# menmitsu/opticalFlowClustering

Measured on AMD Instinct MI355X. Metric: Mpixels/s dense flow+kmeans @1080p, higher is better.
Workload: dtype f32 storage, f64 accumulation; 1 GPU; BASELINE.json configs[2]: 300-frame 1080p synthetic clip, Farneback flow (0.5,3,15,3,5,1.2,0) + Lloyd k=5 over (u,v), frames sharded over 1 GPU(s); width=1920, height=1080, frames=300, pairs=299, k=5, lloyd_iters=11, flow_batch_pairs=64

## Files before the change

include/ofc.h:

```cpp
#ifndef OFC_H
#define OFC_H
#include <stddef.h>
#include <stdint.h>

#ifdef __cplusplus
extern "C" {
#endif

#define OFC_VERSION 100

enum {
    OFC_OK = 0,
    OFC_EINVAL = -1,
    OFC_ENODEV = -2,
    OFC_EHIP = -3,
    OFC_ENOMEM = -4,
    OFC_ENOTREADY = -5,
    OFC_EUNSUPPORTED = -6,
    OFC_ECOMM = -7
};

enum { OFC_U8 = 0, OFC_F32 = 1, OFC_F64 = 2 };

int ofc_version(void);
// ... 15 lines not shown
    int poly_n;
    double poly_sigma;
    int flags;
} ofc_fb_params;
#define OFC_WINSIZE_MAX 255

void ofc_fb_default_params(ofc_fb_params *p);

typedef struct ofc_flow ofc_flow_t;

int ofc_flow_create(int device, int W, int H, const ofc_fb_params *p, int max_batch,
                    ofc_flow_t **out);
void ofc_flow_destroy(ofc_flow_t *f);

int ofc_flow_calc(ofc_flow_t *f, const uint8_t *prev_gray, const uint8_t *next_gray,
                  float *flow_out);

int ofc_flow_calc_frames_dev(ofc_flow_t *f, const uint8_t *frames_dev, int n_frames,
                             float *flow_dev);
int ofc_flow_calc_frames_dev_stats(ofc_flow_t *f, const uint8_t *frames_dev, int n_frames,
                                   float *flow_dev, double *uv_sum_dev);
int ofc_flow_sync(ofc_flow_t *f);
int ofc_flow_front_overlap(const ofc_flow_t *f, int *on);

int ofc_flow_push_gray(ofc_flow_t *f, const uint8_t *gray, float *flow_out);

int ofc_flow_push_bgr(ofc_flow_t *f, const uint8_t *bgr, uint8_t *vis_out, float *mean_mag,
                      float *flow_out);
int ofc_flow_last_vis_dev(ofc_flow_t *f, const uint8_t **vis_dev);

int ofc_level_image(int device, const uint8_t *gray, int W, int H, const ofc_fb_params *p, int k,
                    float *out, int *w_out, int *h_out);
int ofc_polyexp(int device, const float *img, int W, int H, int n, double sigma, float *R5);
int ofc_polyexp_u8(int device, const uint8_t *gray, int W, int H, int n, double sigma, float *R5);
int ofc_update_matrices(int device, const float *R0, const float *R1, const float *flow, int W,
                        int H, float *M);
int ofc_box_solve(int device, const float *M, int W, int H, int winsize, float *flow);
int ofc_flow_resize(int device, const float *flow, int sw, int sh, int dw, int dh, float mul,
                    float *out);

int ofc_flow_iterate(int device, const float *R0, const float *R1, const float *flow_in, int W, int H,
                     int winsize, int iters, int mode, int rows_per_block, float *flow_out);
int ofc_flow_launch_geometry(int W, int H, int n_pairs, int winsize, int out[3]);
int ofc_bench_flow_iters(int device, int W, int H, int n_pairs, int reps, int mode, float *ms);

int ofc_bench_polyexp(int device, int W, int H, int n_images, int iters, int rows_per_block,
                      float *ms_per_launch);

int ofc_bgr2gray(int device, const uint8_t *bgr, int W, int H, uint8_t *gray);
int ofc_flow_to_bgr(int device, const float *flow, int W, int H, uint8_t *bgr, float *mean_mag);
int ofc_flow_to_bgr_dev(int device, const float *flow_dev, int W, int H, int n_frames,
                        uint8_t *bgr_dev, float *mean_mag_dev);
int ofc_bgr2hsv(int device, const uint8_t *bgr, int64_t npix, uint8_t *hsv);
int ofc_preprocess_rgba(int device, const uint8_t *img3, int64_t npix, int thresh, uint8_t *rgba);
int ofc_grid_cell_means(int device, const uint8_t *bgr, int W, int H, int rows, int cols,
// ... 224 lines not shown
```

opticalflowclustering_amd/_lib.py:

```python
import ctypes as C
import os

import numpy as np

_HERE = os.path.dirname(os.path.abspath(__file__))
LIB_PATH = os.path.join(_HERE, "libofc.so")

OFC_OK, OFC_EINVAL, OFC_ENODEV, OFC_EHIP, OFC_ENOMEM, OFC_ENOTREADY, OFC_EUNSUPPORTED, OFC_ECOMM = \
    0, -1, -2, -3, -4, -5, -6, -7
U8, F32, F64 = 0, 1, 2
UNIQUE_ID_BYTES = 128
KPP_CHUNK = 1024
UV_HIST_SHARE = 2048
UV_HIST_MAX_GRID = 2048
BLOB_TILE_W, BLOB_TILE_H, BLOB_FIELDS = 64, 16, 12
BLOB_LINK_FIELDS, BLOB_NO_MOVE = 3, -0x7fff8000
CONSIST_OK, CONSIST_MISMATCH, CONSIST_LEAVES, CONSIST_INVALID, CONSIST_STATES = 0, 1, 2, 3, 4
CONSIST_SHARE, CONSIST_MAX_DIM = 2048, 16384
CONSIST_ALPHA_MAX, CONSIST_BETA_MAX = 65536, 1 << 62
PHOTO_SHARE, PHOTO_TAU_MAX, PHOTO_KAPPA_MAX, PHOTO_NSTAT = 2048, 65280, 1024, 5
REPAIR_ROUNDS_MAX, REPAIR_NCOUNT, REPAIR_UNFILLED = 254, 3, 255


class OfcError(RuntimeError):
# ... 14 lines not shown

_lib = None

_vp, _i, _i64, _f, _d, _sz = C.c_void_p, C.c_int, C.c_int64, C.c_float, C.c_double, C.c_size_t
_ip = C.POINTER(C.c_int)
_PROTOS = {
    "ofc_version": ([], _i),
    "ofc_last_error": ([], C.c_char_p),
    "ofc_device_count": ([_ip], _i),
    "ofc_malloc": ([_i, _sz, C.POINTER(_vp)], _i),
    "ofc_free": ([_i, _vp], _i),
    "ofc_memcpy_h2d": ([_i, _vp, _vp, _sz], _i),
    "ofc_memcpy_d2h": ([_i, _vp, _vp, _sz], _i),
    "ofc_memset": ([_i, _vp, _i, _sz], _i),
    "ofc_device_sync": ([_i], _i),
    "ofc_fb_default_params": ([C.POINTER(FbParams)], None),
    "ofc_flow_create": ([_i, _i, _i, C.POINTER(FbParams), _i, C.POINTER(_vp)], _i),
    "ofc_flow_destroy": ([_vp], None),
    "ofc_flow_calc": ([_vp, _vp, _vp, _vp], _i),
    "ofc_flow_calc_frames_dev": ([_vp, _vp, _i, _vp], _i),
    "ofc_flow_calc_frames_dev_stats": ([_vp, _vp, _i, _vp, _vp], _i),
    "ofc_flow_sync": ([_vp], _i),
    "ofc_flow_front_overlap": ([_vp, _ip], _i),
    "ofc_flow_push_gray": ([_vp, _vp, _vp], _i),
    "ofc_flow_push_bgr": ([_vp, _vp, _vp, C.POINTER(_f), _vp], _i),
    "ofc_flow_last_vis_dev": ([_vp, C.POINTER(_vp)], _i),
    "ofc_level_image": ([_i, _vp, _i, _i, C.POINTER(FbParams), _i, _vp, _ip, _ip], _i),
    "ofc_polyexp": ([_i, _vp, _i, _i, _i, _d, _vp], _i),
    "ofc_polyexp_u8": ([_i, _vp, _i, _i, _i, _d, _vp], _i),
    "ofc_update_matrices": ([_i, _vp, _vp, _vp, _i, _i, _vp], _i),
    "ofc_box_solve": ([_i, _vp, _i, _i, _i, _vp], _i),
    "ofc_flow_resize": ([_i, _vp, _i, _i, _i, _i, _f, _vp], _i),
    "ofc_flow_iterate": ([_i, _vp, _vp, _vp, _i, _i, _i, _i, _i, _i, _vp], _i),
    "ofc_flow_launch_geometry": ([_i, _i, _i, _i, _ip], _i),
    "ofc_bench_flow_iters": ([_i, _i, _i, _i, _i, _i, C.POINTER(_f)], _i),
    "ofc_bench_polyexp": ([_i, _i, _i, _i, _i, _i, C.POINTER(_f)], _i),
    "ofc_bgr2gray": ([_i, _vp, _i, _i, _vp], _i),
    "ofc_flow_to_bgr": ([_i, _vp, _i, _i, _vp, C.POINTER(_f)], _i),
    "ofc_flow_to_bgr_dev": ([_i, _vp, _i, _i, _i, _vp, _vp], _i),
    "ofc_bgr2hsv": ([_i, _vp, _i64, _vp], _i),
    "ofc_preprocess_rgba": ([_i, _vp, _i64, _i, _vp], _i),
    "ofc_grid_cell_means": ([_i, _vp, _i, _i, _i, _i, _vp, _vp], _i),
    "ofc_kmeans_fit": ([_i, _vp, _i, _i64, _i, _i, _vp, _i, _d, _vp, _vp, C.POINTER(_d), _ip], _i),
    "ofc_kmeans_predict": ([_i, _vp, _i, _i64, _i, _i, _vp, _vp], _i),
    "ofc_kmeans_fit_dev": ([_i, _vp, _i, _i64, _i, _i, _vp, _i, _d, _vp, _vp, C.POINTER(_d), _ip], _i),
    "ofc_kmeans_fit_dev_stats": ([_i, _vp, _i, _i64, _i, _i, _vp, _i, _d, _vp, _vp, _vp, C.POINTER(_d), _ip], _i),
    "ofc_kmeans_fit_dev_field": ([_i, _vp, _i, _i64, _i, _i, _vp, _i, _d, _vp, _vp, _vp, C.POINTER(_d), _ip, _i, _i, _i64], _i),
    "ofc_lloyd_field_origin": ([_i64, _i, _i], _i64),
    "ofc_lloyd_field_origins": ([_i64, _i64, _i, _vp], _i),
    "ofc_lloyd_field_shape": ([_ip, _ip, _ip, _ip], None),
    "ofc_lloyd_prune_stats": ([_i, _vp], _i),
    "ofc_bench_lloyd_sweep": ([_i, _vp, _i64, _i, _vp, _vp, _i, _i, C.POINTER(_f)], _i),
    "ofc_lloyd_colstats_dev": ([_i, _vp, _i, _i64, _i, _vp, _i, _vp], _i),
    "ofc_lloyd_step_dev": ([_i, _vp, _i, _i64, _i, _i, _vp, _vp, _vp, _i, _vp], _i),
    "ofc_lloyd_inertia_dev": ([_i, _vp, _i, _i64, _i, _i, _vp, _vp, _vp, C.POINTER(_d)], _i),
    "ofc_lloyd_farthest_dev": ([_i, _vp, _i, _i64, _i, _i, _vp, _vp, _vp, _vp, _i, C.POINTER(_d), C.POINTER(_i64), _vp, _ip], _i),
    "ofc_kmeans_fit_w": ([_i, _vp, _i, _vp, _i, _i64, _i, _i, _vp, _i, _d, _vp, _vp, C.POINTER(_d), _ip], _i),
# ... 157 lines not shown
```

opticalflowclustering_amd/csrc/flow_kernels.hip:

```cpp
#include "flow_device.h"

namespace ofc {

__device__ __forceinline__ void lin_tap_x(int dx, double scale, int sw, int &s0, float &a)
{
#pragma clang fp contract(off)
    float fx = (float)((dx + 0.5) * scale - 0.5);
    int sx = (int)floorf(fx);
    fx -= (float)sx;
    if (sx < 0) { fx = 0.f; sx = 0; }
    if (sx >= sw - 1) { fx = 0.f; sx = sw - 1; }
    s0 = sx;
    a = fx;
}

__device__ __forceinline__ void lin_tap_y(int dy, double scale, int sh, int &s0, int &s1, float &b)
{
#pragma clang fp contract(off)
    float fy = (float)((dy + 0.5) * scale - 0.5);
    int sy = (int)floorf(fy);
    fy -= (float)sy;
    s0 = min(max(sy, 0), sh - 1);
    s1 = min(max(sy + 1, 0), sh - 1);
    b = fy;
// ... 261 lines not shown
int launch_level_image(const uint8_t *src, float *dst, int nimg, int W0, int H0,
                       const LevelGeom &g, hipStream_t s)
{
    LevelArgs a;
    int path = 1;
    size_t lds = 0;
    OFC_TRY(level_image_plan(W0, H0, g, ((uintptr_t)src % 4) == 0, a, path, lds));
    switch (path) {
    case 0:
        hipLaunchKernelGGL(k_level0, dim3(cdiv(W0, 256), cdiv(H0, 32), nimg), dim3(256), 0, s, src, dst, W0, H0,
                           a.kern[0], a.kern[1], a.kern[2]);
        break;
#define OFC_DEC(S_, R_, TX_, TY_)                                                                          \
    case S_:                                                                                               \
        hipLaunchKernelGGL((k_level_dec<S_, R_, TX_, TY_>), dim3(cdiv(g.w, TX_), cdiv(g.h, TY_), nimg),    \
                           dim3(256), 0, s, src, dst, W0, H0, g.w, g.h, a);                                \
        break;
    OFC_DEC(2, 1, 64, 16)
    OFC_DEC(4, 4, 32, 8)
    OFC_DEC(8, 9, 32, 8)
#undef OFC_DEC
    default:
        hipLaunchKernelGGL(k_level_image, dim3(cdiv(g.w, a.txo), cdiv(g.h, a.tyo), nimg), dim3(256), lds, s, src, dst, a);
    }
    OFC_HIP(hipGetLastError());
    return OFC_OK;
}

__device__ __forceinline__ float4 lds_read4(const float *p)
{
    typedef float v4f __attribute__((ext_vector_type(4)));
    typedef const volatile v4f __attribute__((address_space(3))) * lds_v4f_ptr;
    const v4f v = *(lds_v4f_ptr)(p);
    return make_float4(v.x, v.y, v.z, v.w);
}

constexpr int PE_TX = 240;
constexpr int PE_CH = 8;
constexpr int PE_PLANE = 78;

template <int N>
struct PolyArgs {
    int W, H, rows_per_block;
    float g[N + 1], xg[N + 1], xxg[N + 1];
    double ig11, ig03, ig33, ig55;
};
// ... 1104 lines not shown
```

opticalflowclustering_amd/csrc/ofc_api.cpp:

```cpp
#include "color_common.h"
#include "host_util.h"
#include "lloyd_common.h"

#include <cfloat>
#include <algorithm>
#include <cmath>
#include <cstdlib>
#include <memory>

namespace ofc {

static thread_local std::string g_err;

void set_error(const char *fmt, ...)
{
    char buf[1024];
    va_list ap;
    va_start(ap, fmt);
    vsnprintf(buf, sizeof(buf), fmt, ap);
    va_end(ap);
    g_err = buf;
}

int ensure_device(int device)
// ... 175 lines not shown
}

void ofc_fb_default_params(ofc_fb_params *p)
{
    if (!p) return;
    p->pyr_scale = 0.5; p->levels = 3; p->winsize = 15; p->iterations = 3;
    p->poly_n = 5; p->poly_sigma = 1.2; p->flags = 0;
}

}

struct ofc_flow {
    int device = 0, W = 0, H = 0, max_batch = 0, levels = 0;
    ofc_fb_params prm{};
    PolyConsts pc{};
    std::vector<LevelGeom> geom;
    hipStream_t stream = nullptr;
    DevBuf I, R, M, flowA, flowB, flowC;
    bool front_overlap = false;
    hipStream_t side = nullptr;
    hipEvent_t fork = nullptr;
    std::vector<hipEvent_t> ready;
    std::vector<size_t> offI, offR;
    bool fused = true;
    bool fuse_level0 = true;
    bool fuse2 = false;
    int fuse2_min_w = 0;
    bool w3 = false;
    int w3_min_w = 0;
    DevBuf frames2, flow1;
    DevBuf prev_gray;
    bool have_prev = false;
    DevBuf bgr_in, vis, vis_partial, vis_stats, mean_mag;
    bool have_vis = false;
    DevBuf uv_scratch;
    struct Captured {
        const uint8_t *frames = nullptr;
        int n_frames = 0;
        float *flow = nullptr;
        double *uv_sum = nullptr;
        int hits = 0;
        hipGraph_t graph = nullptr;
        hipGraphExec_t exec = nullptr;
    };
    std::vector<Captured> graphs;
    bool use_graph = false;
};

namespace ofc {

static int flow_run(ofc_flow *f, const uint8_t *frames_dev, int n_frames, float *flow_dev, double *uv_sum_dev = nullptr)
{
    const int npair = n_frames - 1;
    const int W = f->W, H = f->H;
    hipStream_t s = f->stream;
    const int iters = f->prm.iterations;
    float *prevFlow = nullptr;
    int pw = 0, ph = 0;
    auto front_end = [&](int k, hipStream_t st) -> int {
        float *I = f->I.as<float>() + f->offI[k], *R = f->R.as<float>() + f->offR[k];
        const LevelGeom &g = f->geom[k];
        if (k == 0 && f->fuse_level0 && polyexp_u8_ok(W, H, g)) return launch_polyexp_u8(frames_dev, R, n_frames, W, H, f->pc, st);
        OFC_TRY(launch_level_image(frames_dev, I, n_frames, W, H, g, st));
        return launch_polyexp(I, R, n_frames, g.w, g.h, f->pc, 0, st);
    };
    if (f->front_overlap) {
        OFC_HIP(hipEventRecord(f->fork, s));
        OFC_HIP(hipStreamWaitEvent(f->side, f->fork, 0));
        for (int k = f->levels; k >= 1; k--) {
            OFC_TRY(front_end(k, f->side));
            OFC_HIP(hipEventRecord(f->ready[k], f->side));
        }
        OFC_TRY(front_end(0, s));
    }
    for (int k = f->levels; k >= 0; k--) {
        const LevelGeom &g = f->geom[k];
        const size_t P = (size_t)g.w * g.h;
        float *dst = (k == 0) ? flow_dev : (((f->levels - k) & 1) ? f->flowB.as<float>() : f->flowA.as<float>());
        float *tmp = f->flowC.as<float>();
        const float *R = f->R.as<float>() + f->offR[k];
        if (!f->front_overlap) {
            OFC_TRY(front_end(k, s));
        } else if (k >= 1) {
            OFC_HIP(hipStreamWaitEvent(s, f->ready[k], 0));
        }
        const size_t strideR = 5 * P;
        const float mul = (float)(1. / f->prm.pyr_scale);
        if (f->fused) {
            const bool two = f->fuse2 && f->prm.winsize == 15 && g.w >= f->fuse2_min_w;
            int plan[64], L = 0;
            for (int i = 0; i < iters;) {
                const int n = (two && i > 0 && iters - i >= 2) ? 2 : 1;
                plan[L++] = n;
// ... 142 lines not shown
    OFC_HIP(hipStreamCreateWithFlags(&f->stream, hipStreamNonBlocking));
    const size_t P0 = (size_t)W * H, nb = (size_t)max_batch;
    size_t nI = P0 * (nb + 1), nR = 5 * P0 * (nb + 1);
    f->offI.assign(f->levels + 1, 0);
    f->offR.assign(f->levels + 1, 0);
    {
        const bool u8_level0 = f->fuse_level0 && polyexp_u8_ok(W, H, f->geom[0]);
        std::vector<size_t> oI(f->levels + 1, 0), oR(f->levels + 1, 0);
        size_t sI = 0, sR = 0;
        for (int k = 0; k <= f->levels; k++) {
            const size_t Pk = (size_t)f->geom[k].w * f->geom[k].h;
            oR[k] = sR;
            sR += (5 * Pk * (nb + 1) + 63) & ~(size_t)63;
            oI[k] = sI;
            if (k > 0 || !u8_level0) sI += (Pk * (nb + 1) + 63) & ~(size_t)63;
        }
        const char *eo = getenv("OFC_FLOW_FRONT_OVERLAP");
        f->front_overlap = !(eo && eo[0] == '0') && f->levels >= 1 && !f->use_graph && 2 * (sI + sR) <= 3 * (nI + nR);
        if (f->front_overlap) {
            f->offI = oI; f->offR = oR;
            nI = sI; nR = sR;
        }
    }
    if (f->front_overlap) {
        OFC_HIP(hipStreamCreateWithFlags(&f->side, hipStreamNonBlocking));
        OFC_HIP(hipEventCreateWithFlags(&f->fork, hipEventDisableTiming));
        f->ready.assign(f->levels + 1, nullptr);
        for (int k = 1; k <= f->levels; k++) OFC_HIP(hipEventCreateWithFlags(&f->ready[k], hipEventDisableTiming));
    }
    OFC_TRY(f->I.alloc(sizeof(float) * nI));
    OFC_TRY(f->R.alloc(sizeof(float) * nR));
    if (f->fused) {
        OFC_TRY(f->flowC.alloc(sizeof(float) * 2 * P0 * nb));
    } else {
        OFC_TRY(f->M.alloc(sizeof(float) * 5 * P0 * nb));
    }
    const size_t P1 = f->levels >= 1 ? (size_t)f->geom[1].w * f->geom[1].h : 1;
    OFC_TRY(f->flowA.alloc(sizeof(float) * 2 * P1 * nb));
    OFC_TRY(f->flowB.alloc(sizeof(float) * 2 * P1 * nb));
    OFC_TRY(f->frames2.alloc(2 * P0));
    OFC_TRY(f->flow1.alloc(sizeof(float) * 2 * P0));
    OFC_TRY(f->prev_gray.alloc(P0));
    *out = f.release();
    return OFC_OK;
}

// ... 30 lines not shown
    OFC_REQUIRE(n_frames >= 2 && n_frames - 1 <= f->max_batch, "n_frames-1 = %d pairs not in [1, max_batch=%d]",
                n_frames - 1, f->max_batch);
    OFC_TRY(ensure_device(f->device));
    return flow_run_cached(f, frames_dev, n_frames, flow_dev, uv_sum_dev);
}

hipStream_t ofc_flow_stream_internal(ofc_flow_t *f) { return f->stream; }

int ofc_flow_sync(ofc_flow_t *f)
{
    OFC_REQUIRE(f, "null pointer");
    OFC_TRY(ensure_device(f->device));
    OFC_HIP(hipStreamSynchronize(f->stream));
    return OFC_OK;
}

int ofc_flow_front_overlap(const ofc_flow_t *f, int *on)
{
    OFC_REQUIRE(f && on, "null pointer");
    *on = f->front_overlap ? 1 : 0;
    return OFC_OK;
}

int ofc_flow_calc(ofc_flow_t *f, const uint8_t *prev_gray, const uint8_t *next_gray, float *flow_out)
{
    OFC_REQUIRE(f && prev_gray && next_gray && flow_out, "null pointer");
    OFC_TRY(ensure_device(f->device));
    const size_t P0 = (size_t)f->W * f->H;
    uint8_t *fr = f->frames2.as<uint8_t>();
    OFC_HIP(hipMemcpyAsync(fr, prev_gray, P0, hipMemcpyHostToDevice, f->stream));
    OFC_HIP(hipMemcpyAsync(fr + P0, next_gray, P0, hipMemcpyHostToDevice, f->stream));
    OFC_TRY(flow_run(f, fr, 2, f->flow1.as<float>()));
    OFC_HIP(hipMemcpyAsync(flow_out, f->flow1.p, sizeof(float) * 2 * P0, hipMemcpyDeviceToHost, f->stream));
    OFC_HIP(hipStreamSynchronize(f->stream));
    return OFC_OK;
}

int ofc_flow_push_gray(ofc_flow_t *f, const uint8_t *gray, float *flow_out)
{
    OFC_REQUIRE(f && gray, "null pointer");
    OFC_TRY(ensure_device(f->device));
    const size_t P0 = (size_t)f->W * f->H;
    uint8_t *fr = f->frames2.as<uint8_t>();
    if (!f->have_prev) {
        OFC_HIP(hipMemcpyAsync(f->prev_gray.p, gray, P0, hipMemcpyHostToDevice, f->stream));
        OFC_HIP(hipStreamSynchronize(f->stream));
// ... 64 lines not shown
{
    for (int c = 0; c < 5; c++)
        for (size_t i = 0; i < P; i++) planar[c * P + i] = inter[i * 5 + c];
}

int ofc_level_image(int device, const uint8_t *gray, int W, int H, const ofc_fb_params *p, int k,
                    float *out, int *w_out, int *h_out)
{
    OFC_REQUIRE(gray && out, "null pointer");
    ofc_fb_params prm;
    if (p) prm = *p; else ofc_fb_default_params(&prm);
    OFC_TRY(check_params(prm, W, H));
    OFC_REQUIRE(k >= 0 && k <= pyramid_levels(W, H, prm), "level %d out of range", k);
    OFC_TRY(ensure_device(device));
    LevelGeom g = level_geometry(W, H, prm, k);
    DevBuf src, dst;
    OFC_TRY(src.alloc((size_t)W * H));
    OFC_TRY(dst.alloc(sizeof(float) * g.w * g.h));
    OFC_HIP(hipMemcpy(src.p, gray, (size_t)W * H, hipMemcpyHostToDevice));
    OFC_TRY(launch_level_image(src.as<uint8_t>(), dst.as<float>(), 1, W, H, g, nullptr));
    OFC_HIP(hipMemcpy(out, dst.p, sizeof(float) * g.w * g.h, hipMemcpyDeviceToHost));
    if (w_out) *w_out = g.w;
    if (h_out) *h_out = g.h;
    return OFC_OK;
}

int ofc_polyexp(int device, const float *img, int W, int H, int n, double sigma, float *R5)
{
    OFC_REQUIRE(img && R5, "null pointer");
    OFC_REQUIRE(W >= 1 && H >= 1, "bad size");
    OFC_TRY(polyexp_n_check(n));
    OFC_TRY(ensure_device(device));
    const size_t P = (size_t)W * H;
    PolyConsts pc;
    polyexp_setup(n, sigma, pc);
    DevBuf I, R;
    OFC_TRY(I.alloc(sizeof(float) * P));
    OFC_TRY(R.alloc(sizeof(float) * 5 * P));
    OFC_HIP(hipMemcpy(I.p, img, sizeof(float) * P, hipMemcpyHostToDevice));
    OFC_TRY(launch_polyexp(I.as<float>(), R.as<float>(), 1, W, H, pc, 0, nullptr));
    OFC_HIP(hipMemcpy(R5, R.p, sizeof(float) * 5 * P, hipMemcpyDeviceToHost));
    return OFC_OK;
}

int ofc_polyexp_u8(int device, const uint8_t *gray, int W, int H, int n, double sigma, float *R5)
{
// ... 171 lines not shown
    PolyConsts pc;
    polyexp_setup(5, 1.2, pc);
    DevBuf I, R;
    OFC_TRY(I.alloc(sizeof(float) * P * n_images));
    OFC_TRY(R.alloc(sizeof(float) * 5 * P * n_images));
    {
        std::vector<float> h(P);
        uint32_t st = 12345u;
        for (int im = 0; im < n_images; im++) {
            for (size_t i = 0; i < P; i++) {
                st = st * 1664525u + 1013904223u;
                h[i] = (float)(st >> 24);
            }
            OFC_HIP(hipMemcpy(I.as<float>() + (size_t)im * P, h.data(), sizeof(float) * P, hipMemcpyHostToDevice));
        }
    }
    ScopedStream own;
    OFC_TRY(own.create());
    hipStream_t s = own.s;
    auto launch = [&]() -> int { return launch_polyexp(I.as<float>(), R.as<float>(), n_images, W, H, pc, rows_per_block, s, true); };
    return time_launches(s, iters, launch, ms_per_launch);
}

}
```

opticalflowclustering_amd/csrc/ofc_common.h:

```cpp
#pragma once
#include <hip/hip_runtime.h>
#include <cstdarg>
#include <cstdint>
#include <cstdio>
#include <cstring>
#include <string>
#include <vector>

#include "../../include/ofc.h"

namespace ofc {

void set_error(const char *fmt, ...);
int ensure_device(int device);

#define OFC_HIP(expr)                                                                         \
    do {                                                                                      \
        hipError_t _e = (expr);                                                               \
        if (_e != hipSuccess) {                                                               \
            ofc::set_error("%s failed: %s (%s:%d)", #expr, hipGetErrorString(_e), __FILE__,   \
                           __LINE__);                                                         \
            return _e == hipErrorOutOfMemory ? OFC_ENOMEM : OFC_EHIP;                         \
        }                                                                                     \
    } while (0)
// ... 37 lines not shown
};

static inline int cdiv(int a, int b) { return (a + b - 1) / b; }
static inline int64_t cdiv64(int64_t a, int64_t b) { return (a + b - 1) / b; }

struct LevelGeom {
    int w, h, ksize;
    double sigma;
};
int pyramid_levels(int W, int H, const ofc_fb_params &p);
LevelGeom level_geometry(int W, int H, const ofc_fb_params &p, int k);
void gaussian_kernel(int n, double sigma, float *k);
struct PolyConsts {
    int n;
    float g[8], xg[8], xxg[8];
    double ig11, ig03, ig33, ig55;
};
void polyexp_setup(int n, double sigma, PolyConsts &c);
int polyexp_n_check(int n);
constexpr int WINSIZE_WIDE_MIN = 19;

int launch_level_image(const uint8_t *src, float *dst, int nimg, int W0, int H0,
                       const LevelGeom &g, hipStream_t s);
bool polyexp_u8_ok(int W, int H, const LevelGeom &g);
int launch_polyexp_u8(const uint8_t *frames, float *R, int nimg, int W, int H, const PolyConsts &c, hipStream_t s);
int launch_polyexp(const float *I, float *R, int nimg, int W, int H, const PolyConsts &c,
                   int rows_per_block, hipStream_t s, bool bench_tag = false);
int launch_update_matrices(const float *R0, const float *R1, size_t pair_stride_R,
                           const float *flow, float *M, int npair, int W, int H, hipStream_t s);
int launch_box_solve(const float *M, float *flow, int npair, int W, int H, int winsize,
                     int rows_per_block, hipStream_t s);
int launch_flow_resize(const float *src, float *dst, int npair, int sw, int sh, int dw, int dh,
                       float mul, hipStream_t s);
int launch_flow_iter(const float *R, size_t frame_stride_R, const float *flow_in, float *flow_out,
                     int npair, int W, int H, int winsize, hipStream_t s, const float *coarse = nullptr,
                     int sw = 0, int sh = 0, float mul = 1.f, double *uv_sum = nullptr, double *uv_scratch = nullptr,
                     size_t uv_scratch_doubles = 0, int rows_per_block = 0);
int flow_iter_rows(int W, int H, int npair, int winsize);
int flow_iter_max_grid(int W, int H, int npair, int winsize);
int launch_flow_iter2(const float *R, size_t frame_stride_R, const float *flow_in, float *flow_out, int npair, int W,
                      int H, int winsize, hipStream_t s, int rows_per_block = 0);
int launch_flow_iter_w3(const float *R, size_t frame_stride_R, const float *flow_in, float *flow_out, int npair, int W,
                        int H, int winsize, hipStream_t s, int rows_per_block = 0);
int launch_flow_iter_pipe(const float *R, size_t frame_stride_R, const float *flow_in, float *flow_out, int npair, int W,
                          int H, int rows_per_block, hipStream_t s, double *uv_sum, double *uv_scratch,
                          size_t uv_scratch_doubles);
// ... 9 lines not shown
```

opticalflowclustering_amd/flow.py:

```python
import ctypes as C
import threading
from collections import OrderedDict

import numpy as np

from . import _lib
from ._lib import FbParams, check, load, ptr


class FlowEngine:

    def __init__(self, W, H, params=None, max_batch=1, device=0):
        self.W, self.H, self.device, self.max_batch = int(W), int(H), device, int(max_batch)
        self.params = params or FbParams()
        h = C.c_void_p()
        check(load().ofc_flow_create(device, self.W, self.H, C.byref(self.params), self.max_batch, C.byref(h)))
        self._h = h

    def calc(self, prev_gray, next_gray, out=None):
        prev_gray = np.ascontiguousarray(prev_gray, np.uint8)
        next_gray = np.ascontiguousarray(next_gray, np.uint8)
        if prev_gray.shape != (self.H, self.W) or next_gray.shape != (self.H, self.W):
            raise ValueError(f"expected two {self.H}x{self.W} uint8 images")
        if out is None:
# ... 9 lines not shown
            raise ValueError(f"expected a {self.H}x{self.W} uint8 image")
        flow = np.empty((self.H, self.W, 2), np.float32)
        rc = load().ofc_flow_push_gray(self._h, ptr(gray), ptr(flow))
        if rc == _lib.OFC_ENOTREADY:
            return None
        check(rc)
        return flow

    def calc_frames_dev(self, frames_ptr, n_frames, flow_ptr, sync=True, uv_sum_ptr=None):
        if uv_sum_ptr:
            check(load().ofc_flow_calc_frames_dev_stats(self._h, C.c_void_p(frames_ptr), n_frames, C.c_void_p(flow_ptr),
                                                        C.c_void_p(uv_sum_ptr)))
        else:
            check(load().ofc_flow_calc_frames_dev(self._h, C.c_void_p(frames_ptr), n_frames, C.c_void_p(flow_ptr)))
        if sync:
            self.sync()

    def sync(self):
        check(load().ofc_flow_sync(self._h))

    def front_overlap(self):
        on = C.c_int(-1)
        check(load().ofc_flow_front_overlap(self._h, C.byref(on)))
        return bool(on.value)

    def close(self):
        if getattr(self, "_h", None):
            load().ofc_flow_destroy(self._h)
            self._h = None

    def __del__(self):
        try:
            self.close()
        except Exception:
            pass


def _is_flow_buffer(a, H, W):
    return (isinstance(a, np.ndarray) and a.dtype == np.float32 and a.shape == (H, W, 2)
            and a.flags.c_contiguous and a.flags.writeable)


OPTFLOW_USE_INITIAL_FLOW = 4
OPTFLOW_FARNEBACK_GAUSSIAN = 256

_FB_CACHE_MAX = 4
# ... 38 lines not shown
```

opticalflowclustering_amd/stages.py:

```python
import ctypes as C

import numpy as np

from ._lib import FbParams, check, load, ptr


def level_image(gray, k, params=None, device=0):
    gray = np.ascontiguousarray(gray, np.uint8)
    H, W = gray.shape
    p = params or FbParams()
    out = np.empty((H, W), np.float32)
    w, h = C.c_int(), C.c_int()
    check(load().ofc_level_image(device, ptr(gray), W, H, C.byref(p), k, ptr(out), C.byref(w), C.byref(h)))
    return out.reshape(-1)[: w.value * h.value].reshape(h.value, w.value).copy()


def polyexp(img, n=5, sigma=1.2, device=0):
    img = np.ascontiguousarray(img, np.float32)
    H, W = img.shape
    out = np.empty((H, W, 5), np.float32)
    check(load().ofc_polyexp(device, ptr(img), W, H, n, sigma, ptr(out)))
    return out


def polyexp_u8(gray, n=5, sigma=1.2, device=0):
    gray = np.ascontiguousarray(gray, np.uint8)
    H, W = gray.shape
    out = np.empty((H, W, 5), np.float32)
    check(load().ofc_polyexp_u8(device, ptr(gray), W, H, n, sigma, ptr(out)))
    return out


def update_matrices(R0, R1, flow, device=0):
    R0, R1, flow = (np.ascontiguousarray(a, np.float32) for a in (R0, R1, flow))
    H, W = flow.shape[:2]
    M = np.empty((H, W, 5), np.float32)
    check(load().ofc_update_matrices(device, ptr(R0), ptr(R1), ptr(flow), W, H, ptr(M)))
# ... 17 lines not shown


def flow_iterate(R0, R1, flow_in, iters, winsize=15, mode=0, rows_per_block=0, device=0):
    R0, R1, flow_in = (np.ascontiguousarray(a, np.float32) for a in (R0, R1, flow_in))
    H, W = flow_in.shape[:2]
    out = np.empty((H, W, 2), np.float32)
    check(load().ofc_flow_iterate(device, ptr(R0), ptr(R1), ptr(flow_in), W, H, winsize, iters, mode, rows_per_block,
                                  ptr(out)))
    return out


def flow_launch_geometry(W, H, n_pairs, winsize=15):
    out = (C.c_int * 3)()
    check(load().ofc_flow_launch_geometry(W, H, n_pairs, winsize, out))
    return tuple(out)


def bench_flow_iters(W, H, n_pairs, reps, mode, device=0):
    ms = C.c_float()
    check(load().ofc_bench_flow_iters(device, W, H, n_pairs, reps, mode, C.byref(ms)))
    return ms.value


def bench_polyexp(W, H, n_images, iters, rows_per_block=0, device=0):
    ms = C.c_float()
    check(load().ofc_bench_polyexp(device, W, H, n_images, iters, rows_per_block, C.byref(ms)))
    return ms.value


def bench_lloyd_sweep(X_ptr, N, centers, mean, what, iters=10, device=0):
    cen = np.ascontiguousarray(centers, np.float64)
    mean = np.ascontiguousarray(mean, np.float64)
    ms = C.c_float()
    check(load().ofc_bench_lloyd_sweep(device, C.c_void_p(X_ptr), N, len(cen), ptr(cen), ptr(mean), what, iters, C.byref(ms)))
    return ms.value


def bench_lloyd_sweep_w(X_ptr, w_ptr, w_dtype, N, centers, mean, iters=10, device=0):
    cen = np.ascontiguousarray(centers, np.float64)
    mean = np.ascontiguousarray(mean, np.float64)
    ms = C.c_float()
    check(load().ofc_bench_lloyd_sweep_w(device, C.c_void_p(X_ptr), C.c_void_p(w_ptr), w_dtype, N, len(cen), ptr(cen), ptr(mean),
                                         iters, C.byref(ms)))
    return ms.value


# ... 12 lines not shown
```

Measured before the change: 19320 Mpixels/s.

## Fuse pyramid level decimations 1..3 into one streaming kernel

Adds a single kernel that reads each u8 frame once and produces the blurred, decimated pyramid levels 1–3 together. It streams vertical bands through LDS ring buffers with separable row and column filters, in place of separate level_image launches per level that each re-read the full-resolution frame. It is enabled by default when front overlap is on and all levels are exact decimations, with an env var to disable it. The side stream then only runs polyexp for those levels. The intent is to cut repeated global reads of the source frames and launch overhead, at the cost of a complex kernel whose LDS use may limit occupancy.

```diff
diff --git a/include/ofc.h b/include/ofc.h
--- a/include/ofc.h
+++ b/include/ofc.h
@@ -61,6 +61,7 @@
                                    float *flow_dev, double *uv_sum_dev);
 int ofc_flow_sync(ofc_flow_t *f);
 int ofc_flow_front_overlap(const ofc_flow_t *f, int *on);
+int ofc_flow_pyramid_fused(const ofc_flow_t *f, int *on);
 
 int ofc_flow_push_gray(ofc_flow_t *f, const uint8_t *gray, float *flow_out);
 
@@ -70,6 +71,10 @@
 
 int ofc_level_image(int device, const uint8_t *gray, int W, int H, const ofc_fb_params *p, int k,
                     float *out, int *w_out, int *h_out);
+int ofc_pyramid_dec(int device, const uint8_t *frames, int n, int W0, int H0, int levels, int fused,
+                    float *out1, float *out2, float *out3, int *fused_levels);
+int ofc_pyramid_dec_geometry(int W0, int H0, int n, int out[4]);
+int ofc_bench_pyramid_dec(int device, int W, int H, int n_images, int levels, int fused, int iters, float *ms_per_batch);
 int ofc_polyexp(int device, const float *img, int W, int H, int n, double sigma, float *R5);
 int ofc_polyexp_u8(int device, const uint8_t *gray, int W, int H, int n, double sigma, float *R5);
 int ofc_update_matrices(int device, const float *R0, const float *R1, const float *flow, int W,
diff --git a/opticalflowclustering_amd/_lib.py b/opticalflowclustering_amd/_lib.py
--- a/opticalflowclustering_amd/_lib.py
+++ b/opticalflowclustering_amd/_lib.py
@@ -60,6 +60,7 @@
     "ofc_flow_calc_frames_dev_stats": ([_vp, _vp, _i, _vp, _vp], _i),
     "ofc_flow_sync": ([_vp], _i),
     "ofc_flow_front_overlap": ([_vp, _ip], _i),
+    "ofc_flow_pyramid_fused": ([_vp, _ip], _i),
     "ofc_flow_push_gray": ([_vp, _vp, _vp], _i),
     "ofc_flow_push_bgr": ([_vp, _vp, _vp, C.POINTER(_f), _vp], _i),
     "ofc_flow_last_vis_dev": ([_vp, C.POINTER(_vp)], _i),
@@ -71,6 +72,9 @@
     "ofc_flow_resize": ([_i, _vp, _i, _i, _i, _i, _f, _vp], _i),
     "ofc_flow_iterate": ([_i, _vp, _vp, _vp, _i, _i, _i, _i, _i, _i, _vp], _i),
     "ofc_flow_launch_geometry": ([_i, _i, _i, _i, _ip], _i),
+    "ofc_pyramid_dec": ([_i, _vp, _i, _i, _i, _i, _i, _vp, _vp, _vp, _ip], _i),
+    "ofc_pyramid_dec_geometry": ([_i, _i, _i, _ip], _i),
+    "ofc_bench_pyramid_dec": ([_i, _i, _i, _i, _i, _i, _i, C.POINTER(_f)], _i),
     "ofc_bench_flow_iters": ([_i, _i, _i, _i, _i, _i, C.POINTER(_f)], _i),
     "ofc_bench_polyexp": ([_i, _i, _i, _i, _i, _i, C.POINTER(_f)], _i),
     "ofc_bgr2gray": ([_i, _vp, _i, _i, _vp], _i),
diff --git a/opticalflowclustering_amd/csrc/flow_kernels.hip b/opticalflowclustering_amd/csrc/flow_kernels.hip
--- a/opticalflowclustering_amd/csrc/flow_kernels.hip
+++ b/opticalflowclustering_amd/csrc/flow_kernels.hip
@@ -307,6 +307,281 @@
 #undef OFC_DEC
     default:
         hipLaunchKernelGGL(k_level_image, dim3(cdiv(g.w, a.txo), cdiv(g.h, a.tyo), nimg), dim3(256), lds, s, src, dst, a);
+    }
+    OFC_HIP(hipGetLastError());
+    return OFC_OK;
+}
+
+struct PyrDecArgs {
+    int W0, H0;
+    int steps, sps;
+    int w[3], h[3];
+    float k1[2], k2[5], k3[10];
+};
+
+constexpr int PD_BAND = 256;
+constexpr int PD_SW = 68;
+
+typedef float pd_v2f __attribute__((ext_vector_type(2)));
+__device__ __forceinline__ pd_v2f pd_ld2(const float2 *p) { const float2 v = *p; return pd_v2f{v.x, v.y}; }
+
+template <int R>
+__device__ __forceinline__ void pd_row_sums(const pd_v2f *b, const float *kh, pd_v2f &a0, pd_v2f &a1)
+{
+#pragma clang fp contract(off)
+    a0 = kh[0] * b[0];
+    a1 = kh[0] * b[1];
+#pragma unroll
+    for (int q = 1; q <= 2 * R; q++) {
+        const float k = kh[q <= R ? q : 2 * R - q];
+        a0 += k * b[q];
+        a1 += k * b[q + 1];
+    }
+}
+
+template <int R>
+__device__ __forceinline__ float pd_col(const pd_v2f *win, const float *kh)
+{
+#pragma clang fp contract(off)
+    float hy[2];
+#pragma unroll
+    for (int yt = 0; yt < 2; yt++) {
+        pd_v2f v = kh[R] * win[R + yt];
+#pragma unroll
+        for (int m = 1; m <= R; m++) v += kh[R - m] * (win[R + yt - m] + win[R + yt + m]);
+        hy[yt] = v.x * 0.5f + v.y * 0.5f;
+    }
+    return hy[0] * 0.5f + hy[1] * 0.5f;
+}
+
+template <int L>
+__global__ __launch_bounds__(256, 4) void k_pyramid_dec(const uint8_t *__restrict__ src, float *__restrict__ dst1,
+                                                     float *__restrict__ dst2, float *__restrict__ dst3, PyrDecArgs p)
+{
+#pragma clang fp contract(off)
+    __shared__ __align__(16) uint32_t stg[8][PD_SW];
+    __shared__ __align__(16) float2 ring1[16][128];
+    __shared__ float2 ring2[L >= 2 ? 16 : 1][64];
+    __shared__ float2 ring3[L >= 3 ? 24 : 1][32];
+    const int tid = threadIdx.x, W0 = p.W0, H0 = p.H0;
+    const int band = blockIdx.x, x0 = band * PD_BAND;
+    const int t0 = blockIdx.y * p.sps, t1 = min(p.steps, t0 + p.sps);
+    const bool first = t0 == 0, last = t1 == p.steps;
+    const uint8_t *img = src + (size_t)blockIdx.z * W0 * H0;
+    const int lo1 = first ? 0 : 4 * t0 + 3, hi1 = last ? p.h[0] : min(p.h[0], 4 * t1 + 3);
+    const int lo2 = first ? 0 : 2 * t0 + 1, hi2 = last ? p.h[1] : min(p.h[1], 2 * t1 + 1);
+    const int hi3 = min(p.h[2], t1);
+    float *out1 = dst1 + (size_t)blockIdx.z * p.w[0] * p.h[0];
+    float *out2 = L >= 2 ? dst2 + (size_t)blockIdx.z * p.w[1] * p.h[1] : nullptr;
+    float *out3 = L >= 3 ? dst3 + (size_t)blockIdx.z * p.w[2] * p.h[2] : nullptr;
+
+    int srow[3], scol[3], smode[3];
+#pragma unroll
+    for (int n = 0; n < 3; n++) {
+        const int s = min(tid + 256 * n, 8 * PD_SW - 1);
+        srow[n] = s / PD_SW;
+        const int c = s - srow[n] * PD_SW;
+        scol[n] = x0 - 8 + 4 * c;
+        smode[n] = (scol[n] >= 0 && scol[n] + 4 <= W0) ? 0 : (scol[n] < W0 + 8 ? 1 : 2);
+    }
+    const bool third = tid < 8 * PD_SW - 512;
+    uint32_t d[3];
+    auto fetch = [&](int t) {
+#pragma unroll
+        for (int n = 0; n < 3; n++) {
+            if (n == 2 && !third) break;
+            const int v = 8 * t + 7 + srow[n];
+            int y = v < 0 ? -v : (v >= H0 ? 2 * (H0 - 1) - v : v);
+            y = min(max(y, 0), H0 - 1);
+            const uint8_t *row = img + (size_t)y * W0;
+            if (smode[n] == 0) {
+                d[n] = *reinterpret_cast<const uint32_t *>(row + scol[n]);
+            } else if (smode[n] == 1) {
+                uint32_t w = 0;
+#pragma unroll
+                for (int e = 0; e < 4; e++) {
+                    const int x = scol[n] + e, xr = x < 0 ? -x : (x >= W0 ? 2 * (W0 - 1) - x : x);
+                    w |= (uint32_t)row[min(max(xr, 0), W0 - 1)] << (8 * e);
+                }
+                d[n] = w;
+            } else {
+                d[n] = 0;
+            }
+        }
+    };
+
+    auto step = [&](auto phc, int t, bool rows12, bool col12, bool col3) {
+        constexpr int PH = decltype(phc)::value, P2 = PH % 2, P3 = PH % 3;
+        if (tid < 128) {
+            if constexpr (L >= 3) {
+                const int j = tid & 31, r = tid >> 5;
+                uint32_t wd[2][6];
+#pragma unroll
+                for (int i = 0; i < 2; i++) {
+                    const uint2 *w2 = reinterpret_cast<const uint2 *>(&stg[r + 4 * i][2 * j]);
+                    const uint2 wa = w2[0], wb = w2[1], wc = w2[2];
+                    wd[i][0] = wa.x; wd[i][1] = wa.y; wd[i][2] = wb.x; wd[i][3] = wb.y; wd[i][4] = wc.x; wd[i][5] = wc.y;
+                }
+                pd_v2f b[20], a0, a1;
+#pragma unroll
+                for (int q = 0; q < 20; q++)
+                    b[q] = pd_v2f{ubyte_of(wd[0][(2 + q) >> 2], (2 + q) & 3), ubyte_of(wd[1][(2 + q) >> 2], (2 + q) & 3)};
+                pd_row_sums<9>(b, p.k3, a0, a1);
+                ring3[P3 * 8 + r][j] = make_float2(a0.x, a1.x);
+                ring3[P3 * 8 + r + 4][j] = make_float2(a0.y, a1.y);
+            }
+        } else if (rows12) {
+            if constexpr (L >= 2) {
+                const int j = tid & 63, r = (tid >> 6) & 1;
+#pragma unroll
+                for (int h = 0; h < 2; h++) {
+                    uint32_t wd[2][3];
+#pragma unroll
+                    for (int i = 0; i < 2; i++) {
+                        const uint32_t *w1 = &stg[r + 2 * h + 4 * i][j + 1];
+                        wd[i][0] = w1[0]; wd[i][1] = w1[1]; wd[i][2] = w1[2];
+                    }
+                    pd_v2f b[10], a0, a1;
+#pragma unroll
+                    for (int q = 0; q < 10; q++)
+                        b[q] = pd_v2f{ubyte_of(wd[0][(1 + q) >> 2], (1 + q) & 3), ubyte_of(wd[1][(1 + q) >> 2], (1 + q) & 3)};
+                    pd_row_sums<4>(b, p.k2, a0, a1);
+                    ring2[P2 * 8 + r + 2 * h][j] = make_float2(a0.x, a1.x);
+                    ring2[P2 * 8 + r + 2 * h + 4][j] = make_float2(a0.y, a1.y);
+                }
+            }
+        }
+        if (rows12) {
+            const int c = tid & 63, r = tid >> 6;
+            uint32_t wd[2][3];
+#pragma unroll
+            for (int i = 0; i < 2; i++) {
+                const uint32_t *w1 = &stg[r + 4 * i][c + 1];
+                wd[i][0] = w1[0]; wd[i][1] = w1[1]; wd[i][2] = w1[2];
+            }
+            pd_v2f b[6], a0[2], a1[2];
+#pragma unroll
+            for (int q = 0; q < 6; q++)
+                b[q] = pd_v2f{ubyte_of(wd[0][(3 + q) >> 2], (3 + q) & 3), ubyte_of(wd[1][(3 + q) >> 2], (3 + q) & 3)};
+#pragma unroll
+            for (int e = 0; e < 2; e++) pd_row_sums<1>(b + 2 * e, p.k1, a0[e], a1[e]);
+            *reinterpret_cast<float4 *>(&ring1[P2 * 8 + r][2 * c]) = make_float4(a0[0].x, a1[0].x, a0[1].x, a1[1].x);
+            *reinterpret_cast<float4 *>(&ring1[P2 * 8 + r + 4][2 * c]) = make_float4(a0[0].y, a1[0].y, a0[1].y, a1[1].y);
+        }
+        __syncthreads();
+        if (tid < 128) {
+            const int ox = 128 * band + tid;
+            if (col12 && ox < p.w[0]) {
+                pd_v2f win[10];
+#pragma unroll
+                for (int q = 0; q < 10; q++) win[q] = pd_ld2(&ring1[(P2 * 8 + q - 2 + 16) % 16][tid]);
+#pragma unroll
+                for (int a = 0; a < 4; a++) {
+                    const int oy = 4 * t + 3 + a;
+                    const float v = pd_col<1>(win + 2 * a, p.k1);
+                    if (oy >= lo1 && oy < hi1) out1[(size_t)oy * p.w[0] + ox] = v;
+                }
+            }
+        } else if (tid < 192) {
+            if constexpr (L >= 2) {
+                const int j = tid - 128, ox = 64 * band + j;
+                if (col12 && ox < p.w[1]) {
+                    pd_v2f win[14];
+#pragma unroll
+                    for (int q = 0; q < 14; q++) win[q] = pd_ld2(&ring2[(P2 * 8 + q - 6 + 16) % 16][j]);
+#pragma unroll
+                    for (int a = 0; a < 2; a++) {
+                        const int oy = 2 * t + 1 + a;
+                        const float v = pd_col<4>(win + 4 * a, p.k2);
+                        if (oy >= lo2 && oy < hi2) out2[(size_t)oy * p.w[1] + ox] = v;
+                    }
+                }
+            }
+        } else if (tid < 224) {
+            if constexpr (L >= 3) {
+                const int j = tid - 192, ox = 32 * band + j;
+                if (col3 && t < hi3 && ox < p.w[2]) {
+                    pd_v2f win[20];
+#pragma unroll
+                    for (int q = 0; q < 20; q++) win[q] = pd_ld2(&ring3[(P3 * 8 + q - 13 + 24) % 24][j]);
+                    out3[(size_t)t * p.w[2] + ox] = pd_col<9>(win, p.k3);
+                }
+            }
+        }
+    };
+
+    const int tb = (L >= 3 || (L >= 2 && first)) ? t0 - 2 : t0 - 1;
+    int ph = (tb + 6) % 6;
+    fetch(tb);
+    for (int t = tb; t < t1; t++) {
+#pragma unroll
+        for (int n = 0; n < 3; n++)
+            if (n < 2 || third) stg[srow[n]][(scol[n] - x0 + 8) >> 2] = d[n];
+        __syncthreads();
+        if (t + 1 < t1) fetch(t + 1);
+        const bool rows12 = t >= t0 - 1 || t < 0, col12 = t >= t0 || t == -1, col3 = t >= t0;
+        switch (ph) {
+        case 0: step(std::integral_constant<int, 0>{}, t, rows12, col12, col3); break;
+        case 1: step(std::integral_constant<int, 1>{}, t, rows12, col12, col3); break;
+        case 2: step(std::integral_constant<int, 2>{}, t, rows12, col12, col3); break;
+        case 3: step(std::integral_constant<int, 3>{}, t, rows12, col12, col3); break;
+        case 4: step(std::integral_constant<int, 4>{}, t, rows12, col12, col3); break;
+        default: step(std::integral_constant<int, 5>{}, t, rows12, col12, col3); break;
+        }
+        ph = ph == 5 ? 0 : ph + 1;
+    }
+}
+
+void pyramid_dec_plan(int W0, int H0, int nimg, int &bands, int &steps, int &sps, int &strips)
+{
+    bands = cdiv(W0, PD_BAND);
+    steps = cdiv(H0, 8);
+    const int64_t nb = std::max<int64_t>(1, (int64_t)nimg * bands);
+    const int want = (int)std::max<int64_t>(1, (1024 + nb / 2) / nb);
+    sps = std::max(4, cdiv(steps, want));
+    strips = cdiv(steps, sps);
+}
+
+int pyramid_dec_levels(int W0, int H0, const LevelGeom *geom, int levels, bool src_aligned)
+{
+    static const int want[3] = {2, 4, 8};
+    int n = 0;
+    for (int k = 1; k <= std::min(levels, 3); k++) {
+        LevelArgs a;
+        int path = 1;
+        size_t lds = 0;
+        if (level_image_plan(W0, H0, geom[k], src_aligned, a, path, lds) != OFC_OK || path != want[k - 1]) break;
+        n = k;
+    }
+    return n;
+}
+
+int launch_pyramid_dec(const uint8_t *src, float *const *dst, int nimg, int W0, int H0, const LevelGeom *geom, int L,
+                       hipStream_t s)
+{
+    OFC_REQUIRE(L >= 1 && L <= 3 && pyramid_dec_levels(W0, H0, geom, L, ((uintptr_t)src % 4) == 0) == L,
+                "k_pyramid_dec: levels 1..%d of %d x %d are not all exact decimations", L, W0, H0);
+    PyrDecArgs p;
+    memset(&p, 0, sizeof(p));
+    p.W0 = W0; p.H0 = H0;
+    int bands, strips;
+    pyramid_dec_plan(W0, H0, nimg, bands, p.steps, p.sps, strips);
+    for (int k = 1; k <= L; k++) {
+        LevelArgs a;
+        int path = 1;
+        size_t lds = 0;
+        OFC_TRY(level_image_plan(W0, H0, geom[k], true, a, path, lds));
+        p.w[k - 1] = geom[k].w; p.h[k - 1] = geom[k].h;
+        for (int q = 0; q < a.r; q++)
+            OFC_REQUIRE(a.kern[q] == a.kern[2 * a.r - q], "k_pyramid_dec: level %d's kernel is not symmetric", k);
+        memcpy(k == 1 ? p.k1 : k == 2 ? p.k2 : p.k3, a.kern, sizeof(float) * (a.r + 1));
+    }
+    const dim3 grid(bands, strips, nimg);
+    float *d1 = dst[0], *d2 = L >= 2 ? dst[1] : nullptr, *d3 = L >= 3 ? dst[2] : nullptr;
+    switch (L) {
+    case 1: hipLaunchKernelGGL(k_pyramid_dec<1>, grid, dim3(256), 0, s, src, d1, d2, d3, p); break;
+    case 2: hipLaunchKernelGGL(k_pyramid_dec<2>, grid, dim3(256), 0, s, src, d1, d2, d3, p); break;
+    default: hipLaunchKernelGGL(k_pyramid_dec<3>, grid, dim3(256), 0, s, src, d1, d2, d3, p);
     }
     OFC_HIP(hipGetLastError());
     return OFC_OK;
diff --git a/opticalflowclustering_amd/csrc/ofc_api.cpp b/opticalflowclustering_amd/csrc/ofc_api.cpp
--- a/opticalflowclustering_amd/csrc/ofc_api.cpp
+++ b/opticalflowclustering_amd/csrc/ofc_api.cpp
@@ -221,6 +221,7 @@
     hipEvent_t fork = nullptr;
     std::vector<hipEvent_t> ready;
     std::vector<size_t> offI, offR;
+    bool pyramid_fused = false;
     bool fused = true;
     bool fuse_level0 = true;
     bool fuse2 = false;
@@ -266,8 +267,19 @@
     if (f->front_overlap) {
         OFC_HIP(hipEventRecord(f->fork, s));
         OFC_HIP(hipStreamWaitEvent(f->side, f->fork, 0));
+        const bool one_launch = f->pyramid_fused && ((uintptr_t)frames_dev % 4) == 0;
+        if (one_launch) {
+            float *lv[3] = {nullptr, nullptr, nullptr};
+            for (int k = 1; k <= f->levels; k++) lv[k - 1] = f->I.as<float>() + f->offI[k];
+            OFC_TRY(launch_pyramid_dec(frames_dev, lv, n_frames, W, H, f->geom.data(), f->levels, f->side));
+        }
         for (int k = f->levels; k >= 1; k--) {
-            OFC_TRY(front_end(k, f->side));
+            if (one_launch) {
+                const LevelGeom &g = f->geom[k];
+                OFC_TRY(launch_polyexp(f->I.as<float>() + f->offI[k], f->R.as<float>() + f->offR[k], n_frames, g.w, g.h, f->pc, 0, f->side));
+            } else {
+                OFC_TRY(front_end(k, f->side));
+            }
             OFC_HIP(hipEventRecord(f->ready[k], f->side));
         }
         OFC_TRY(front_end(0, s));
@@ -456,6 +468,11 @@
             nI = sI; nR = sR;
         }
     }
+    {
+        const char *ep = getenv("OFC_PYRAMID_FUSED");
+        f->pyramid_fused = !(ep && ep[0] == '0') && f->front_overlap && f->levels <= 3 &&
+                           pyramid_dec_levels(W, H, f->geom.data(), f->levels, true) == f->levels;
+    }
     if (f->front_overlap) {
         OFC_HIP(hipStreamCreateWithFlags(&f->side, hipStreamNonBlocking));
         OFC_HIP(hipEventCreateWithFlags(&f->fork, hipEventDisableTiming));
@@ -532,6 +549,13 @@
     return OFC_OK;
 }
 
+int ofc_flow_pyramid_fused(const ofc_flow_t *f, int *on)
+{
+    OFC_REQUIRE(f && on, "null pointer");
+    *on = f->pyramid_fused ? 1 : 0;
+    return OFC_OK;
+}
+
 int ofc_flow_calc(ofc_flow_t *f, const uint8_t *prev_gray, const uint8_t *next_gray, float *flow_out)
 {
     OFC_REQUIRE(f && prev_gray && next_gray && flow_out, "null pointer");
@@ -642,6 +666,46 @@
     OFC_HIP(hipMemcpy(out, dst.p, sizeof(float) * g.w * g.h, hipMemcpyDeviceToHost));
     if (w_out) *w_out = g.w;
     if (h_out) *h_out = g.h;
+    return OFC_OK;
+}
+
+int ofc_pyramid_dec(int device, const uint8_t *frames, int n, int W0, int H0, int levels, int fused,
+                    float *out1, float *out2, float *out3, int *fused_levels)
+{
+    OFC_REQUIRE(frames && out1 && (levels < 2 || out2) && (levels < 3 || out3), "null pointer");
+    OFC_REQUIRE(n >= 1 && levels >= 1 && levels <= 3, "n >= 1 frames and 1..3 levels");
+    ofc_fb_params prm;
+    ofc_fb_default_params(&prm);
+    prm.levels = levels;
+    OFC_TRY(check_params(prm, W0, H0));
+    std::vector<LevelGeom> geom;
+    for (int k = 0; k <= levels; k++) {
+        geom.push_back(level_geometry(W0, H0, prm, k));
+        OFC_REQUIRE(geom[k].w >= 1 && geom[k].h >= 1, "level %d of %d x %d is empty", k, W0, H0);
+    }
+    OFC_TRY(ensure_device(device));
+    float *outs[3] = {out1, out2, out3};
+    DevBuf src, dst[3];
+    OFC_TRY(src.alloc((size_t)n * W0 * H0));
+    for (int k = 1; k <= levels; k++) OFC_TRY(dst[k - 1].alloc(sizeof(float) * n * geom[k].w * geom[k].h));
+    OFC_HIP(hipMemcpy(src.p, frames, (size_t)n * W0 * H0, hipMemcpyHostToDevice));
+    const int L = fused ? pyramid_dec_levels(W0, H0, geom.data(), levels, true) : 0;
+    if (L >= 1) {
+        float *lv[3] = {dst[0].as<float>(), dst[1].as<float>(), dst[2].as<float>()};
+        OFC_TRY(launch_pyramid_dec(src.as<uint8_t>(), lv, n, W0, H0, geom.data(), L, nullptr));
+    }
+    for (int k = L + 1; k <= levels; k++)
+        OFC_TRY(launch_level_image(src.as<uint8_t>(), dst[k - 1].as<float>(), n, W0, H0, geom[k], nullptr));
+    for (int k = 1; k <= levels; k++)
+        OFC_HIP(hipMemcpy(outs[k - 1], dst[k - 1].p, sizeof(float) * n * geom[k].w * geom[k].h, hipMemcpyDeviceToHost));
+    if (fused_levels) *fused_levels = L;
+    return OFC_OK;
+}
+
+int ofc_pyramid_dec_geometry(int W0, int H0, int n, int *out4)
+{
+    OFC_REQUIRE(out4 && W0 >= 1 && H0 >= 1 && n >= 1, "bad arguments");
+    pyramid_dec_plan(W0, H0, n, out4[0], out4[1], out4[2], out4[3]);
     return OFC_OK;
 }
 
@@ -859,4 +923,45 @@
     return time_launches(s, iters, launch, ms_per_launch);
 }
 
-}
+int ofc_bench_pyramid_dec(int device, int W, int H, int n_images, int levels, int fused, int iters, float *ms_per_batch)
+{
+    OFC_REQUIRE(ms_per_batch && n_images >= 1 && iters >= 1 && levels >= 1 && levels <= 3, "bad arguments");
+    ofc_fb_params prm;
+    ofc_fb_default_params(&prm);
+    prm.levels = levels;
+    OFC_TRY(check_params(prm, W, H));
+    std::vector<LevelGeom> geom;
+    for (int k = 0; k <= levels; k++) geom.push_back(level_geometry(W, H, prm, k));
+    if (fused && pyramid_dec_levels(W, H, geom.data(), levels, true) != levels) {
+        set_error("levels 1..%d of %d x %d are not all exact decimations", levels, W, H);
+        return OFC_EUNSUPPORTED;
+    }
+    OFC_TRY(ensure_device(device));
+    const size_t P = (size_t)W * H;
+    DevBuf src, dst[3];
+    OFC_TRY(src.alloc(P * n_images));
+    for (int k = 1; k <= levels; k++) OFC_TRY(dst[k - 1].alloc(sizeof(float) * n_images * geom[k].w * geom[k].h));
+    {
+        std::vector<uint8_t> h(P);
+        uint32_t st = 12345u;
+        for (int im = 0; im < n_images; im++) {
+            for (size_t i = 0; i < P; i++) {
+                st = st * 1664525u + 1013904223u;
+                h[i] = (uint8_t)(st >> 24);
+            }
+            OFC_HIP(hipMemcpy(src.as<uint8_t>() + (size_t)im * P, h.data(), P, hipMemcpyHostToDevice));
+        }
+    }
+    ScopedStream own;
+    OFC_TRY(own.create());
+    hipStream_t s = own.s;
+    float *lv[3] = {dst[0].as<float>(), dst[1].as<float>(), dst[2].as<float>()};
+    auto launch = [&]() -> int {
+        if (fused) return launch_pyramid_dec(src.as<uint8_t>(), lv, n_images, W, H, geom.data(), levels, s);
+        for (int k = levels; k >= 1; k--) OFC_TRY(launch_level_image(src.as<uint8_t>(), lv[k - 1], n_images, W, H, geom[k], s));
+        return OFC_OK;
+    };
+    return time_launches(s, iters, launch, ms_per_batch);
+}
+
+}
diff --git a/opticalflowclustering_amd/csrc/ofc_common.h b/opticalflowclustering_amd/csrc/ofc_common.h
--- a/opticalflowclustering_amd/csrc/ofc_common.h
+++ b/opticalflowclustering_amd/csrc/ofc_common.h
@@ -83,6 +83,10 @@
 
 int launch_level_image(const uint8_t *src, float *dst, int nimg, int W0, int H0,
                        const LevelGeom &g, hipStream_t s);
+int pyramid_dec_levels(int W0, int H0, const LevelGeom *geom, int levels, bool src_aligned);
+void pyramid_dec_plan(int W0, int H0, int nimg, int &bands, int &steps, int &sps, int &strips);
+int launch_pyramid_dec(const uint8_t *src, float *const *dst, int nimg, int W0, int H0, const LevelGeom *geom, int L,
+                       hipStream_t s);
 bool polyexp_u8_ok(int W, int H, const LevelGeom &g);
 int launch_polyexp_u8(const uint8_t *frames, float *R, int nimg, int W, int H, const PolyConsts &c, hipStream_t s);
 int launch_polyexp(const float *I, float *R, int nimg, int W, int H, const PolyConsts &c,
diff --git a/opticalflowclustering_amd/flow.py b/opticalflowclustering_amd/flow.py
--- a/opticalflowclustering_amd/flow.py
+++ b/opticalflowclustering_amd/flow.py
@@ -55,6 +55,11 @@
     def front_overlap(self):
         on = C.c_int(-1)
         check(load().ofc_flow_front_overlap(self._h, C.byref(on)))
+        return bool(on.value)
+
+    def pyramid_fused(self):
+        on = C.c_int(-1)
+        check(load().ofc_flow_pyramid_fused(self._h, C.byref(on)))
         return bool(on.value)
 
     def close(self):
diff --git a/opticalflowclustering_amd/stages.py b/opticalflowclustering_amd/stages.py
--- a/opticalflowclustering_amd/stages.py
+++ b/opticalflowclustering_amd/stages.py
@@ -13,6 +13,22 @@
     w, h = C.c_int(), C.c_int()
     check(load().ofc_level_image(device, ptr(gray), W, H, C.byref(p), k, ptr(out), C.byref(w), C.byref(h)))
     return out.reshape(-1)[: w.value * h.value].reshape(h.value, w.value).copy()
+
+
+def pyramid_dec(frames, levels, fused=True, device=0):
+    frames = np.ascontiguousarray(frames, np.uint8)
+    n, H, W = frames.shape
+    outs = [np.empty((n, int(np.rint(H * 0.5 ** k)), int(np.rint(W * 0.5 ** k))), np.float32) for k in range(1, levels + 1)]
+    ptrs = [ptr(o) for o in outs] + [None] * (3 - levels)
+    nf = C.c_int(-1)
+    check(load().ofc_pyramid_dec(device, ptr(frames), n, W, H, levels, int(bool(fused)), *ptrs, C.byref(nf)))
+    return outs, nf.value
+
+
+def pyramid_dec_geometry(W, H, n):
+    out = (C.c_int * 4)()
+    check(load().ofc_pyramid_dec_geometry(W, H, n, out))
+    return tuple(out)
 
 
 def polyexp(img, n=5, sigma=1.2, device=0):
@@ -76,6 +92,12 @@
     return ms.value
 
 
+def bench_pyramid_dec(W, H, n_images, levels=3, fused=True, iters=20, device=0):
+    ms = C.c_float()
+    check(load().ofc_bench_pyramid_dec(device, W, H, n_images, levels, int(bool(fused)), iters, C.byref(ms)))
+    return ms.value
+
+
 def bench_polyexp(W, H, n_images, iters, rows_per_block=0, device=0):
     ms = C.c_float()
     check(load().ofc_bench_polyexp(device, W, H, n_images, iters, rows_per_block, C.byref(ms)))
```

Measured after the change: 19610 Mpixels/s (median of 6 runs). 1.02x the previous value.
